# lzzcd001/MeshDiffusion

Hardware: NVIDIA H100
Metric: denoising sample-steps/sec at res-64 (4x64^3), uncond_gen PC sampler (higher is better)
Workload: dtype bf16x3

## Files before the change

### meshdiffusion_b200/csrc/gemm_host.cu

```cuda
#include "gemm_host.h"
#include "elementwise.cuh"
#include <cstring>
#include <cstdlib>
#include <mutex>

namespace mdb {

typedef CUresult (*PFN_encodeTiled)(CUtensorMap*, CUtensorMapDataType, cuuint32_t, void*, const cuuint64_t*,
                                    const cuuint64_t*, const cuuint32_t*, const cuuint32_t*, CUtensorMapInterleave,
                                    CUtensorMapSwizzle, CUtensorMapL2promotion, CUtensorMapFloatOOBfill);

static PFN_encodeTiled get_encode() {
  static PFN_encodeTiled fn = nullptr;
  static std::once_flag once;
  std::call_once(once, [] {
    void* f = nullptr;
    cudaDriverEntryPointQueryResult q;
    cudaError_t e = cudaGetDriverEntryPoint("cuTensorMapEncodeTiled", &f, cudaEnableDefault, &q);
    if (e != cudaSuccess || q != cudaDriverEntryPointSuccess || !f)
      throw std::runtime_error("mdb: cuTensorMapEncodeTiled not available (needs an sm_90+ driver)");
    fn = reinterpret_cast<PFN_encodeTiled>(f);
  });
  return fn;
}
// ... 104 lines not shown
  if (by > 16) by = 16;
  if (by > Y) by = Y;
  int rem = 128 / (bx * by);
  int bz = rem < Z ? rem : Z;
  int bb = rem / bz;
  return {bx, by, bz, bb};
}

int plan_splits(int X, int Y, int Z, int B, int N, int cin_total, int taps, Precision prec) {
  const Geometry g = pick_geometry(X, Y, Z);
  const int tiles_m = ((X + g.bx - 1) / g.bx) * ((Y + g.by - 1) / g.by) * ((Z + g.bz - 1) / g.bz) * ((B + g.bb - 1) / g.bb);
  const int block_n = N <= 32 ? 32 : 128;
  const int tiles = tiles_m * ((N + block_n - 1) / block_n);
  const int kprod = ((cin_total + kb_elems(prec) - 1) / kb_elems(prec)) * taps * (prec == kBF16X3 ? 3 : 1);
  if (tiles > 49 || kprod < 48) return 1;
  int S = kPlanSMs / tiles;
  if (S > 16) S = 16;
  if (S > kprod / 8) S = kprod / 8;
  return S < 2 ? 1 : S;
}

void GemmOp::enable_splits(int S, float* scratch) {
  if (S <= 1) return;
  if (p.ocs != 1 || p.out_fp32 || p.bias_on_m || p.alpha != 1.f || p.res_fp32)
    throw std::runtime_error("mdb: split-K is only wired for plain NDHWC conv outputs");
  if (p.osx != (long long)p.N * parts(prec) || (p.rsx && p.rsx != (long long)p.N * parts(prec)))
    throw std::runtime_error("mdb: split-K needs dense [B][V][N] output / residual");
  splits = S;
  p.splits = S;
  p.partial = scratch;
  p.split_stride = (long long)p.Bn * p.X * p.Y * p.Z * p.N;
}

GemmOp::~GemmOp() {
  if (d_loads) cudaFree(d_loads);
  if (d_ks0) cudaFree(d_ks0);
  if (d_wpacked && owns_w) cudaFree(d_wpacked);
}

static long long physical_strides(bool split, long long lo_off, long long& sx, long long& sy, long long& sz, long long& sb) {
  if (!split) return 0;
  sx *= 2; sy *= 2; sz *= 2; sb *= 2;
  return lo_off;
}

void GemmOp::set_output_strided(Precision pr, int X, int Y, int Z, int B, int N, void* out, long long osx,
                                long long osy, long long osz, long long osb, bool out_fp32, long long lo_off) {
  prec = pr;
  geo = pick_geometry(X, Y, Z);
  if (geo.bx * geo.by * geo.bz * geo.bb != kBlockM) throw std::runtime_error("mdb: unsupported tile geometry");
  if (geo.bb > 1 && (geo.bx * geo.by * geo.bz) % 32 != 0)
    throw std::runtime_error("mdb: multi-sample tiles need a multiple of 32 rows per sample");
  if (geo.bb > 4) throw std::runtime_error("mdb: at most 4 samples per tile");
  p.bx = geo.bx; p.by = geo.by; p.bz = geo.bz; p.bb = geo.bb;
  p.X = X; p.Y = Y; p.Z = Z; p.Bn = B;
  p.tx = (X + geo.bx - 1) / geo.bx; p.ty = (Y + geo.by - 1) / geo.by;
  p.tz = (Z + geo.bz - 1) / geo.bz; p.tb = (B + geo.bb - 1) / geo.bb;
  p.N = N;
  block_n = N <= 32 ? 32 : 128;
  p.n_tiles_n = (N + block_n - 1) / block_n;
  p.out = out;
  p.osx = osx; p.osy = osy; p.osz = osz; p.osb = osb;
  p.out_fp32 = out_fp32 ? 1 : 0;
  p.out_lo_off = physical_strides(prec == kBF16X3 && !out_fp32, lo_off >= 0 ? lo_off : osx, p.osx, p.osy, p.osz, p.osb);
  p.alpha = 1.f;
  p.ocs = 1;
  p.kb_elems = kb_elems(prec);
// ... 267 lines not shown
    p.b_explicit_k = 1;
    p.b_lo_k = (int)b_lo_off;
  }
  if (!b_from_act) p.b_batched = 0;
  p.n_loads = (int)loads.size();
  if (p.splits < 1) p.splits = 1;
  {
    a_slot_need = 0;
    nk_max = 0;
    p.n_segs = 0;
    p.total_groups = 0;
    size_t i = 0;
    while (i < loads.size()) {
      size_t j = i;
      while (j < loads.size() && loads[j].nk == loads[i].nk && loads[j].rows == loads[i].rows && loads[j].jrows == loads[i].jrows) ++j;
      if (p.n_segs >= kMaxSegs) throw std::runtime_error("mdb: too many pipeline segments");
      GemmSeg sg{};
      sg.n_groups = (int)(j - i); sg.nk = loads[i].nk;
      sg.a_bytes = loads[i].rows * kRowBytes;
      sg.a_stride = (sg.a_bytes + 1023) / 1024 * 1024;
      sg.jbytes = loads[i].jrows * kRowBytes;
      const int need = parts(prec) * sg.a_stride;
      if (sg.a_stride > kAStageBytes) throw std::runtime_error("mdb: A box exceeds the slot size");
      if (need > a_slot_need) a_slot_need = need;
      if (sg.nk > nk_max) nk_max = sg.nk;
      p.segs[p.n_segs++] = sg;
      p.total_groups += sg.n_groups;
      i = j;
    }
  }
  if (p.splits > p.total_groups) { p.splits = p.total_groups; splits = p.splits; }
}

void GemmOp::upload(cudaStream_t stream) {
  for (size_t i = 0; i < amaps_.size(); ++i) encode_map(&p.amap[i], prec, amaps_[i]);
  MDB_CUDA_CHECK(cudaMalloc(&d_loads, loads.size() * sizeof(LoadEntry)));
  MDB_CUDA_CHECK(cudaMemcpyAsync(d_loads, loads.data(), loads.size() * sizeof(LoadEntry), cudaMemcpyHostToDevice, stream));
  p.loads = d_loads;
  if (!b_from_act) {
    const long long ktot = 1LL * ksteps * kb_elems(prec) * parts(prec);
    const long long bytes = ktot * p.N * esize(prec);
    MDB_CUDA_CHECK(cudaMalloc(&d_wpacked, bytes));
    owns_w = true;
    bmap_ = b_desc(d_wpacked, ktot, p.N, 1, ktot * esize(prec), bytes);
  }
  encode_map(&p.bmap, prec, bmap_);
  MDB_CUDA_CHECK(cudaStreamSynchronize(stream));
}

void GemmOp::launch(cudaStream_t stream, int B, void* out_override) const {
  GemmParams p = this->p;
  const int smem = pick_slots(p);
  if (B > 0) {
    if (B > this->p.Bn) throw std::runtime_error("mdb: batch exceeds the batch the op was built for");
    p.Bn = B;
    p.tb = (B + p.bb - 1) / p.bb;
  }
  if (out_override) p.out = out_override;
  const int tiles_m = p.tx * p.ty * p.tz * p.tb;
  const int total = tiles_m * p.n_tiles_n * (p.splits > 1 ? p.splits : 1);
  const int grid = total < sm_count() ? total : sm_count();
  if (gnb) {
    if (p.splits > 1) throw std::runtime_error("mdb: GroupNorm-backward epilogue: no split-K");
    p.gnb_drop_thresh = rt_drop_thresh; p.gnb_drop_scale = rt_drop_scale; p.gnb_seed = rt_seed;
  }
  gemm_variant(block_n, prec, gnb).launch(p, grid, smem, stream);
  if (p.splits > 1) {
    SplitReduceArgs a{};
    a.partial = p.partial; a.split_stride = p.split_stride; a.splits = p.splits;
    a.bias = p.bias; a.rowbias = p.rowbias; a.rowbias_ld = p.rowbias_ld;
    a.res = p.res; a.res_batch_stride = p.rsb;
    a.out = p.out; a.stats = p.stats; a.voxels = (long long)p.X * p.Y * p.Z; a.N = p.N; a.prec = prec;
    if (prec == kBF16X3) a.res_batch_stride = p.rsb / 2;
    launch_split_reduce(a, p.Bn, stream);
  }
}

}
```

### meshdiffusion_b200/csrc/gemm_host.h

```cpp
#pragma once
#include <cuda.h>
#include <cuda_runtime.h>
#include <stdint.h>
#include <string>
#include <vector>
#include <stdexcept>
#include "act_format.cuh"
#include "gemm_tc.cuh"

namespace mdb {

#define MDB_CUDA_CHECK(expr)                                                                         \
  do {                                                                                               \
    cudaError_t _e = (expr);                                                                         \
    if (_e != cudaSuccess)                                                                           \
      throw std::runtime_error(std::string("CUDA error ") + cudaGetErrorString(_e) + " at " + __FILE__ + ":" + \
                               std::to_string(__LINE__) + " (" #expr ")");                           \
  } while (0)

inline int kb_elems(Precision p) { return kRowBytes / esize(p); }

struct Act {
  void* ptr = nullptr;
  int C = 0, X = 0, Y = 0, Z = 0, B = 0;
// ... 7 lines not shown
  const float* ptr = nullptr;
  long long sn = 0, sc = 0, st = 0;
  int cvalid = 0;
  int ndiv = 0;
  long long sn_hi = 0;
  int cdiv = 0;
  long long sc_hi = 0;
};

struct Geometry { int bx, by, bz, bb; };
Geometry pick_geometry(int X, int Y, int Z);

struct MapDesc {
  void* base = nullptr;
  int rank = 0;
  uint64_t dims[5] = {}, strides[4] = {};
  uint32_t box[5] = {};
};
MapDesc act_map(const Act& a, Precision prec, int part, Geometry box, int sub = 1, int px = 0, int py = 0, int pz = 0);

class GemmOp {
 public:
  GemmParams p{};
  Precision prec = kBF16;
  int block_n = 128;
  int splits = 1;
  std::vector<LoadEntry> loads;
  std::vector<WSrc> wsrcs;
  int ksteps = 0;
  LoadEntry* d_loads = nullptr;
  int* d_ks0 = nullptr;
  void* d_wpacked = nullptr;
  bool owns_w = false;
  double flops = 0;
  std::string name;

  ~GemmOp();
  GemmOp() = default;
  GemmOp(const GemmOp&) = delete;
  GemmOp& operator=(const GemmOp&) = delete;

  void set_output(Precision prec, int X, int Y, int Z, int B, int N, void* out, long long ldc, bool out_fp32);
  void set_output_strided(Precision prec, int X, int Y, int Z, int B, int N, void* out, long long osx, long long osy,
                          long long osz, long long osb, bool out_fp32, long long lo_off = -1);
  int add_amap(const Act& a, int halo_rows_y, int sub_stride = 1, int px = 0, int py = 0, int pz = 0, int part = 0);
  void add_load_x(int tm_hi, int tm_lo, int nk, int rows, int jrows, int dx, int dy, int dz, int c0, int wsrc, int wc0,
                  int tap0, int tapj);
  int add_wsrc(const WSrc& w) { wsrcs.push_back(w); return (int)wsrcs.size() - 1; }

  void add_conv(const std::vector<Act>& srcs, const float* w_oidhw, int ksize, int stride);
  void add_conv_w(const std::vector<Act>& srcs, const WSrc& w, int ksize, int stride);
  void add_conv_up2(const Act& src, const float* w8, int px, int py, int pz);
  void add_conv_dgrad(const Act& dy, const float* w_oidhw, int cin_total, int ksize);
  void add_pointwise(const std::vector<Act>& srcs, const float* w, bool w_in_out);
  void add_pointwise_w(const std::vector<Act>& srcs, const WSrc* w);

  void set_b_activation(void* ptr, int K, int N, int batch, long long row_stride_elems, long long batch_stride_elems);

  void set_bias(const float* bias, bool on_m = false) { p.bias = bias; p.bias_on_m = on_m ? 1 : 0; }
  void set_rowbias(const float* rb, long long ld) { p.rowbias = rb; p.rowbias_ld = ld; }
  void set_out_col_stride(long long ocs) { p.ocs = ocs; }
  void set_residual(const void* res, long long ldr, long long batch_stride, bool fp32);
  void set_stats(long long* stats) { p.stats = stats; }
  void set_gn_backward(const void* x0, long long ld0, int c0, const void* x1, long long ld1, const void* consts, int silu, float* part);
  long long gnb_rows() const { return 1LL * p.tx * p.ty * p.tz * p.tb * p.bb; }
  int gnb_tiles_per_batch_tile() const { return p.tx * p.ty * p.tz; }
  int gnb_bb() const { return p.bb; }
  bool gnb = false;
  int rt_drop_thresh = 0; float rt_drop_scale = 1.f; unsigned long long rt_seed = 0;
  void set_alpha(float a) { p.alpha = a; }
  void enable_splits(int S, float* scratch);

  void finalize();
  void upload(cudaStream_t stream);
  void repack(cudaStream_t stream);
  void launch(cudaStream_t stream, int B = -1, void* out_override = nullptr) const;
  double fill_bytes(int B = -1) const;
  void slots(int& a_slots, int& b_slots, int& smem_bytes) const;

 private:
  Geometry geo{};
  bool b_from_act = false;
  int a_slot_need = 0;
  int nk_max = 0;
  int pick_slots(GemmParams& q) const;
  long long b_lo_off = 0;
  std::vector<MapDesc> amaps_;
  MapDesc bmap_;
  MapDesc b_desc(void* ptr, long long K, int N, int batch, long long row_stride_bytes, long long batch_stride_bytes) const;
};

int sm_count();
constexpr int kPlanSMs = 132;
void encode_map(CUtensorMap* m, Precision prec, const MapDesc& d);
int plan_splits(int X, int Y, int Z, int B, int N, int cin_total, int taps, Precision prec);

}
```

### meshdiffusion_b200/csrc/gemm_tc.cuh

```cuda
#pragma once
#include "ptx.cuh"
#include "act_format.cuh"
#include "gn_stats.cuh"

namespace mdb {

constexpr int kBlockM = 128;
constexpr int kRowBytes = 128;
constexpr int kAStageRows = 160;
constexpr int kAStageBytes = kAStageRows * kRowBytes;
constexpr int kMaxLoads = 2048;
constexpr int kMaxAMaps = 16;
constexpr int kGemmThreads = 384;
constexpr int kEpiThreads = 256;

struct __align__(16) LoadEntry {
  uint8_t tmap;
  uint8_t nk;
  uint8_t rows;
  uint8_t jrows;
  int8_t dx, dy, dz;
  uint8_t wsrc;
  uint16_t c0;
  uint16_t wc0;
  uint8_t tap0;
  uint8_t tapj;
  uint8_t tmap_lo;
  uint8_t pad;
};
static_assert(sizeof(LoadEntry) == 16, "LoadEntry must be 16 bytes");

struct GemmSeg {
  int n_groups;
  int nk;
  int a_bytes;
  int a_stride;
  int jbytes;
};
constexpr int kMaxSegs = 8;

struct GemmParams {
  CUtensorMap amap[kMaxAMaps];
  CUtensorMap bmap;
  const LoadEntry* loads;
  int n_loads;
  int n_segs;
  GemmSeg segs[kMaxSegs];
  int bx, by, bz, bb;
  int X, Y, Z, Bn;
  int tx, ty, tz, tb;
  int n_tiles_n;
  int N;
  int b_batched;
  int splits;
  int total_groups;
  float* partial;
  long long split_stride;
  int batch_fastest;
  int kb_elems;
  int b_explicit_k;
  int b_kstep;
  int b_lo_k;
  int n_aslots, a_slot_bytes, n_bslots, b_slot_bytes;
  long long out_lo_off, res_lo_off;
  void* out;
  long long osx, osy, osz, osb;
  long long ocs;
  int out_fp32;
  const float* bias;
  int bias_on_m;
  const float* rowbias;
  long long rowbias_ld;
  const void* res;
  long long rsx, rsy, rsz, rsb;
  int res_fp32;
  float alpha;
  long long* stats;
  const void* res1;
  long long r1sx, r1sy, r1sz, r1sb;
  long long res1_lo_off;
  int res_c0;
  const float4* gnb_c;
  int gnb_silu;
  int gnb_drop_thresh; float gnb_drop_scale; unsigned long long gnb_seed;
  float* gnb_part;
};

constexpr int kMaxSlots = 8;
constexpr int kMaxDynSmem = 232448;
template <int BLOCK_N, bool kWholeTile = false>
struct GemmCfg {
  static constexpr int kBTileBytes = BLOCK_N * kRowBytes;
  static constexpr int kStatsFloats = 24 * BLOCK_N;
  static constexpr int kStageCols = (kWholeTile || BLOCK_N < 64) ? BLOCK_N : 64;
  static constexpr int kStageRounds = BLOCK_N / kStageCols;
  static_assert(kStageRounds <= 2, "the epilogue stages at most two rounds");
  static constexpr int kAccPitch = kStageCols + 4;
  static constexpr int kAccFloats = kBlockM * kAccPitch;
  static constexpr int kFixedBytes = 1024 + kAccFloats * 4 + kStatsFloats * 4 + 4 * kMaxSlots * 8;
};
constexpr int kRegsProducer = 40, kRegsConsumer = 232;

__device__ __forceinline__ uint64_t kdesc(uint32_t saddr) { return make_wgmma_desc(saddr, 16, 1024); }

template <int OFF>
__device__ __forceinline__ void colsum_butterfly(float (&s)[32], float (&ss)[32], int lane) {
  const bool hi = (lane & OFF) != 0;
#pragma unroll
  for (int i = 0; i < OFF; ++i) {
    const float send_s = hi ? s[i] : s[i + OFF];
    const float send_q = hi ? ss[i] : ss[i + OFF];
    const float keep_s = hi ? s[i + OFF] : s[i];
    const float keep_q = hi ? ss[i + OFF] : ss[i];
    s[i] = keep_s + __shfl_xor_sync(0xffffffffu, send_s, OFF);
    ss[i] = keep_q + __shfl_xor_sync(0xffffffffu, send_q, OFF);
  }
  if constexpr (OFF > 1) colsum_butterfly<OFF / 2>(s, ss, lane);
}

template <Precision P>
__device__ __forceinline__ void add_res_chunk(const uint4 (&buf)[8], float (&v)[32]) {
  constexpr int E = kVecElems<P>, NV = 32 / E;
#pragma unroll
  for (int i = 0; i < NV; ++i) {
    float r[E];
    decode_vec<P>(buf[i], buf[P == kBF16X3 ? NV + i : i], r);
#pragma unroll
    for (int j = 0; j < E; ++j) v[E * i + j] += r[j];
  }
}

template <int BLOCK_N, Precision P, bool GNB>
__global__ void __launch_bounds__(kGemmThreads, 1) gemm_tc_kernel(const __grid_constant__ GemmParams p) {
  static_assert(!(GNB && P == kTF32), "the GroupNorm-backward epilogue is built for bf16 / split-bf16 operands");
  using Cfg = GemmCfg<BLOCK_N, GNB>;
// ... 65 lines not shown
          const GemmSeg& seg = p.segs[sg];
          for (int g = 0; g < seg.n_groups; ++g, ++gi) {
            if (gi < g_lo || gi >= g_hi) {
              kcol += seg.nk * p.b_kstep;
              ++l;
              continue;
            }
            const uint4 raw = __ldg(reinterpret_cast<const uint4*>(p.loads + l));
            const LoadEntry& en = reinterpret_cast<const LoadEntry&>(raw);
            mbar_wait(a_empty + 8 * as, aph ^ 1);
            if (elect_one()) {
              const uint32_t abase = a_ring + as * a_slot, bar = a_full + 8 * as;
              mbar_expect_tx(bar, kParts * seg.a_bytes);
              tma_load_5d(&p.amap[en.tmap], bar, abase, en.c0, x0 + en.dx, y0 + en.dy, z0 + en.dz, b0);
              if constexpr (P == kBF16X3) tma_load_5d(&p.amap[en.tmap_lo], bar, abase + seg.a_stride, en.c0, x0 + en.dx, y0 + en.dy, z0 + en.dz, b0);
            }
            __syncwarp();
            if (++as == (uint32_t)NA) { as = 0; aph ^= 1; }
            int kc = (P == kBF16X3 && p.b_explicit_k) ? (int)en.wc0 : kcol;
            for (int j = 0; j < seg.nk; ++j) {
              mbar_wait(b_empty + 8 * bs, bph ^ 1);
              if (elect_one()) {
                const uint32_t bbase = b_ring + bs * b_slot, bar = b_full + 8 * bs;
                mbar_expect_tx(bar, kParts * Cfg::kBTileBytes);
                tma_load_3d(&p.bmap, bar, bbase, kc, n0, bcoord);
                if constexpr (P == kBF16X3) tma_load_3d(&p.bmap, bar, bbase + Cfg::kBTileBytes, kc + p.b_lo_k, n0, bcoord);
              }
              __syncwarp();
              kc += p.b_kstep;
              if (++bs == (uint32_t)NB) { bs = 0; bph ^= 1; }
            }
            kcol += seg.nk * p.b_kstep;
            ++l;
          }
        }
      }
    }
  } else {
    setmaxnreg_inc<kRegsConsumer>();
    const int wg = (warp - 4) >> 2;
    const int wt = threadIdx.x & 127;
    const int q = warp & 3;
    const int half = (warp - 4) >> 2;
    constexpr int kChunks = BLOCK_N / 32;
    constexpr int kChunkStep = kChunks >= 2 ? 2 : 1;
    const int row = q * 32 + lane;
    const int et = threadIdx.x - 128;
    const int rows_per_b = p.bx * p.by * p.bz;
    const int seg = row / rows_per_b;
    int it = 0;
    int staged_n0 = -1, staged_b0 = -1, bias_buf = 0;
    int want_cols = 0;
    if constexpr (GNB) {
      want_cols = (p.stats != nullptr || p.gnb_part != nullptr) ? 1 : 0;
      asm volatile("" : "+r"(want_cols));
    }
    uint32_t as = 0, aph = 0, bs = 0, bph = 0;
    for (int tile = first_tile; tile < total_tiles; tile += tile_step, ++it) {
      const int vit = it;
      constexpr int kAccRegs = kParts * BLOCK_N / 2;
      float acc[kAccRegs];
      float (&acc_hi)[BLOCK_N / 2] = *reinterpret_cast<float (*)[BLOCK_N / 2]>(acc);
#pragma unroll
      for (int i = 0; i < kAccRegs; ++i) acc[i] = 0.f;
      {
        int gi = 0, g_lo, g_hi;
        split_range(tile, g_lo, g_hi);
        int prev_b = -1, prev_a = -1;
        const uint32_t a_row0 = (uint32_t)wg * 64 * kRowBytes;
        for (int sg = 0; sg < p.n_segs; ++sg) {
          const GemmSeg& sgm = p.segs[sg];
          for (int g = 0; g < sgm.n_groups; ++g, ++gi) {
            if (gi < g_lo || gi >= g_hi) continue;
            mbar_wait(a_full + 8 * as, aph);
            const uint32_t abase = a_ring + as * a_slot + a_row0;
            for (int j = 0; j < sgm.nk; ++j) {
              mbar_wait(b_full + 8 * bs, bph);
              const uint64_t ad = kdesc(abase + j * sgm.jbytes);
              const uint64_t bd = kdesc(b_ring + bs * b_slot);
              wgmma_fence();
              if constexpr (P == kBF16X3) {
                const uint64_t adl = kdesc(abase + sgm.a_stride + j * sgm.jbytes);
#pragma unroll
                for (int k = 0; k < kRowBytes / 32; ++k) wgmma_kmajor<2 * BLOCK_N, false>(acc, ad + 2 * k, bd + 2 * k, 1u);
                wgmma_fence();
#pragma unroll
                for (int k = 0; k < kRowBytes / 32; ++k) wgmma_kmajor<BLOCK_N, false>(acc_hi, adl + 2 * k, bd + 2 * k, 1u);
              } else {
#pragma unroll
                for (int k = 0; k < kRowBytes / 32; ++k) wgmma_kmajor<BLOCK_N, P == kTF32>(acc, ad + 2 * k, bd + 2 * k, 1u);
              }
              wgmma_commit();
              wgmma_wait<1>();
              if (wt == 0) {
                if (prev_b >= 0) mbar_arrive(b_empty + 8 * prev_b);
                if (prev_a >= 0) mbar_arrive(a_empty + 8 * prev_a);
              }
              prev_b = (int)bs;
              prev_a = j + 1 == sgm.nk ? (int)as : -1;
              if (++bs == (uint32_t)NB) { bs = 0; bph ^= 1; }
            }
            if (++as == (uint32_t)NA) { as = 0; aph ^= 1; }
          }
        }
        wgmma_wait<0>();
        fence_operands(acc);
        if (wt == 0) {
          if (prev_b >= 0) mbar_arrive(b_empty + 8 * prev_b);
          if (prev_a >= 0) mbar_arrive(a_empty + 8 * prev_a);
        }
        if constexpr (P == kBF16X3) {
#pragma unroll
          for (int i = 0; i < BLOCK_N / 2; ++i) acc[i] += acc[BLOCK_N / 2 + i];
        }
      }
      int x0, y0, z0, b0, n0;
      decode(tile, x0, y0, z0, b0, n0);
      int r = row;
      const int xl = r % p.bx; r /= p.bx;
      const int yl = r % p.by; r /= p.by;
      const int zl = r % p.bz; r /= p.bz;
      const int xg = x0 + xl, yg = y0 + yl, zg = z0 + zl, bg = b0 + r;
      const bool valid = (xg < p.X) && (yg < p.Y) && (zg < p.Z) && (bg < p.Bn);
      const long long ooff = xg * p.osx + yg * p.osy + zg * p.osz + bg * p.osb;
      const long long roff = xg * p.rsx + yg * p.rsy + zg * p.rsz + bg * p.rsb;

      constexpr int kRoundRegs = Cfg::kStageCols / 2;
      auto stage = [&]() {
        const int w4 = (warp & 3), srow = wg * 64 + w4 * 16 + (lane >> 2), scol = 2 * (lane & 3);
#pragma unroll
        for (int j = 0; j < Cfg::kStageCols / 8; ++j) {
          *reinterpret_cast<float2*>(s_acc + srow * Cfg::kAccPitch + 8 * j + scol) = make_float2(acc[4 * j], acc[4 * j + 1]);
          *reinterpret_cast<float2*>(s_acc + (srow + 8) * Cfg::kAccPitch + 8 * j + scol) = make_float2(acc[4 * j + 2], acc[4 * j + 3]);
        }
      };
      named_bar_sync(2, kEpiThreads);
      stage();
      if constexpr (Cfg::kStageRounds > 1) {
#pragma unroll
// ... 21 lines not shown
      uint4 rbuf[8];
      auto prefetch_res = [&](int ch) {
        const int nbp = n0 + ch * 32;
        if (!(p.res && valid && p.ocs == 1 && nbp + 32 <= p.N)) return;
        if constexpr (GNB) {
          const bool second = p.res1 && nbp >= p.res_c0;
          const __nv_bfloat16* base = reinterpret_cast<const __nv_bfloat16*>(second ? p.res1 : p.res);
          const long long off = second ? xg * p.r1sx + yg * p.r1sy + zg * p.r1sz + bg * p.r1sb + (nbp - p.res_c0) : roff + nbp;
          const uint4* rp = reinterpret_cast<const uint4*>(base + off);
#pragma unroll
          for (int i = 0; i < 4; ++i) rbuf[i] = __ldg(rp + i);
          if constexpr (P == kBF16X3) {
            const uint4* rl = reinterpret_cast<const uint4*>(base + off + (second ? p.res1_lo_off : p.res_lo_off));
#pragma unroll
            for (int i = 0; i < 4; ++i) rbuf[4 + i] = __ldg(rl + i);
          }
          return;
        }
        if (P == kTF32 || p.res_fp32) {
          const uint4* rp = reinterpret_cast<const uint4*>(reinterpret_cast<const float*>(p.res) + roff + nbp);
#pragma unroll
          for (int i = 0; i < 8; ++i) rbuf[i] = __ldg(rp + i);
        } else {
          const uint4* rp = reinterpret_cast<const uint4*>(reinterpret_cast<const __nv_bfloat16*>(p.res) + roff + nbp);
#pragma unroll
          for (int i = 0; i < 4; ++i) rbuf[i] = __ldg(rp + i);
          if constexpr (P == kBF16X3) {
            const uint4* rl = reinterpret_cast<const uint4*>(reinterpret_cast<const __nv_bfloat16*>(p.res) + roff + nbp + p.res_lo_off);
#pragma unroll
            for (int i = 0; i < 4; ++i) rbuf[4 + i] = __ldg(rl + i);
          }
        }
      };
      const int ch0 = kChunkStep == 2 ? half : 0;
      const bool active = kChunkStep == 2 || half == 0;
      if (active) prefetch_res(ch0);

      constexpr int kRoundChunks = Cfg::kStageCols / 32;
#pragma unroll 1
      for (int rnd = 0; rnd < Cfg::kStageRounds; ++rnd) {
        if (rnd > 0) {
          named_bar_sync(2, kEpiThreads);
          stage();
        }
        named_bar_sync(2, kEpiThreads);

#pragma unroll 1
        for (int ch = ch0 + rnd * kRoundChunks; ch < (rnd + 1) * kRoundChunks && active; ch += kChunkStep) {
          uint32_t rr[32];
          {
            const float4* src = reinterpret_cast<const float4*>(s_acc + row * Cfg::kAccPitch + (ch - rnd * kRoundChunks) * 32);
#pragma unroll
            for (int i = 0; i < 8; ++i) {
              const float4 t = src[i];
              rr[4 * i] = __float_as_uint(t.x); rr[4 * i + 1] = __float_as_uint(t.y);
              rr[4 * i + 2] = __float_as_uint(t.z); rr[4 * i + 3] = __float_as_uint(t.w);
            }
          }
          const int nb = n0 + ch * 32;
          if (nb >= p.N) continue;
          if (splits > 1) {
            if (valid) {
              float* pp = p.partial + (long long)(tile % splits) * p.split_stride + (P == kBF16X3 ? (ooff >> 1) : ooff) + nb;
              if (nb + 32 <= p.N) {
#pragma unroll
                for (int i = 0; i < 8; ++i)
                  reinterpret_cast<float4*>(pp)[i] = make_float4(__uint_as_float(rr[4 * i]), __uint_as_float(rr[4 * i + 1]),
                                                                 __uint_as_float(rr[4 * i + 2]), __uint_as_float(rr[4 * i + 3]));
              } else {
                for (int i = 0; i < 32; ++i) if (nb + i < p.N) pp[i] = __uint_as_float(rr[i]);
              }
            }
            continue;
          }
          const bool full = (nb + 32 <= p.N) && (p.ocs == 1);
          float v[32];
          const float mbias = (p.bias && p.bias_on_m && valid) ? __ldg(p.bias + xg) : 0.f;
          const float* sb = s_bias + (seg < 4 ? seg : 0) * BLOCK_N + ch * 32;
// ... 2 lines not shown
          float q2[GNB ? 32 : 1];
          if constexpr (GNB) {
            if (valid) {
              const float4* cc = p.gnb_c + static_cast<long long>(bg) * p.N + nb;
              unsigned long long hsh[8];
              if (p.gnb_drop_thresh > 0) {
                const unsigned long long e4 = (unsigned long long)((((static_cast<long long>(bg) * p.Z + zg) * p.Y + yg) * p.X + xg) * p.N + nb) >> 2;
#pragma unroll
                for (int i = 0; i < 8; ++i) hsh[i] = drop_hash64(p.gnb_seed, e4 + i);
              }
#pragma unroll
              for (int i = 0; i < 32; ++i) {
                const float4 kc = __ldg(cc + i);
                const __nv_bfloat16 xb = reinterpret_cast<const __nv_bfloat16*>(rbuf)[i];
                float xv = __bfloat162float(xb);
                if constexpr (P == kBF16X3) xv += __bfloat162float(reinterpret_cast<const __nv_bfloat16*>(rbuf + 4)[i]);
                float d = v[i];
                if (p.gnb_drop_thresh > 0) {
                  const unsigned r16 = (unsigned)((hsh[i >> 2] >> (16 * (i & 3))) & 0xFFFFu);
                  d = r16 >= (unsigned)p.gnb_drop_thresh ? d * p.gnb_drop_scale : 0.f;
                }
                if (p.gnb_silu) {
                  const float h = fmaf(xv, kc.x, kc.y);
                  d *= P == kBF16X3 ? dsilu_ex2_half(h) : dsilu_tanh_half(h);
                }
                v[i] = d;
                q2[i] = d * fmaf(xv, kc.z, kc.w);
              }
            } else {
#pragma unroll
              for (int i = 0; i < 32; ++i) q2[i] = 0.f;
            }
          }
          if (!GNB && p.res && valid) {
            if (P == kTF32 || p.res_fp32) {
              if (full) {
                add_res_chunk<kTF32>(rbuf, v);
              } else {
                const float* rp = reinterpret_cast<const float*>(p.res) + roff + nb;
                for (int i = 0; i < 32; ++i) if (nb + i < p.N) v[i] += rp[i];
              }
            } else {
              if (full) {
                add_res_chunk<P>(rbuf, v);
              } else {
                const ActElem<P>* rp = reinterpret_cast<const ActElem<P>*>(p.res) + roff + nb;
                for (int i = 0; i < 32; ++i) if (nb + i < p.N) v[i] += load_split<P>(rp + i, p.res_lo_off);
              }
            }
          }
          if (ch + kChunkStep < kChunks) prefetch_res(ch + kChunkStep);
          if (valid) {
            if (p.out_fp32) {
              float* op = reinterpret_cast<float*>(p.out) + ooff + nb;
              if (full) {
#pragma unroll
                for (int i = 0; i < 8; ++i) reinterpret_cast<float4*>(op)[i] = make_float4(v[4 * i], v[4 * i + 1], v[4 * i + 2], v[4 * i + 3]);
              } else {
                for (int i = 0; i < 32; ++i) if (nb + i < p.N) op[i * p.ocs] = v[i];
              }
            } else {
              ActElem<P>* op = reinterpret_cast<ActElem<P>*>(p.out) + ooff + nb;
              if (full) {
                constexpr int E = kVecElems<P>;
#pragma unroll
                for (int i = 0; i < 32 / E; ++i) store_vec<P>(op + E * i, p.out_lo_off * (long long)sizeof(ActElem<P>), v + E * i);
              } else {
                for (int i = 0; i < 32; ++i) if (nb + i < p.N) store_split<P>(op + i * p.ocs, p.out_lo_off, v[i]);
              }
            }
          }
          if (GNB ? (want_cols != 0) : (p.stats != nullptr)) {
            float s[32], ss[32];
#pragma unroll
            for (int i = 0; i < 32; ++i) {
              const float t = valid ? v[i] : 0.f;
              s[i] = t; ss[i] = GNB ? q2[GNB ? i : 0] : t * t;
            }
            colsum_butterfly<16>(s, ss, lane);
            s_part[(q * 2 + 0) * BLOCK_N + ch * 32 + lane] = s[0];
            s_part[(q * 2 + 1) * BLOCK_N + ch * 32 + lane] = ss[0];
          }
        }
      }
      if constexpr (GNB) {
        if (p.gnb_part && splits == 1) {
          named_bar_sync(1, kEpiThreads);
          const int warps_per_seg = rows_per_b >= 128 ? 4 : rows_per_b / 32;
          for (int i = et; i < p.bb * BLOCK_N; i += kEpiThreads) {
            const int sg = i / BLOCK_N, c = i % BLOCK_N;
            const int n = n0 + c;
            if (mt_of_tile < tiles_m && n < p.N) {
              float ts = 0.f, tq = 0.f;
              for (int w = sg * warps_per_seg; w < (sg + 1) * warps_per_seg; ++w) {
                ts += s_part[(w * 2 + 0) * BLOCK_N + c];
                tq += s_part[(w * 2 + 1) * BLOCK_N + c];
              }
              float* dst = p.gnb_part + ((static_cast<long long>(mt_of_tile) * p.bb + sg) * p.N + n) * 2;
              dst[0] = ts; dst[1] = tq;
            }
          }
        }
      }
      if (!GNB && p.stats && splits == 1) {
        named_bar_sync(1, kEpiThreads);
        const int warps_per_seg = rows_per_b >= 128 ? 4 : rows_per_b / 32;
        for (int i0 = 0; i0 < p.bb * BLOCK_N; i0 += kEpiThreads) {
          const int i = i0 + et;
          const int sg = i / BLOCK_N, c = i % BLOCK_N;
          const int bgl = b0 + sg, n = n0 + c;
          if (i < p.bb * BLOCK_N && bgl < p.Bn && n < p.N) {
            float ts = 0.f, tq = 0.f;
            for (int w = sg * warps_per_seg; w < (sg + 1) * warps_per_seg; ++w) {
              ts += s_part[(w * 2 + 0) * BLOCK_N + c];
              tq += s_part[(w * 2 + 1) * BLOCK_N + c];
            }
            long long* dst = p.stats + (static_cast<long long>(bgl) * p.N + n) * kStatWords;
            stat_add(dst, ts);
            stat_add(dst + 2, tq);
          }
        }
      }
    }
  }
}

}
```

### meshdiffusion_b200/csrc/ptx.cuh

```cuda
#pragma once
#include <cuda.h>
#include <cuda_runtime.h>
#include <cuda_bf16.h>
#include <stdint.h>
#include <stdio.h>

namespace mdb {

__device__ __forceinline__ uint32_t smem_u32(const void* p) {
  return static_cast<uint32_t>(__cvta_generic_to_shared(p));
}

__device__ __forceinline__ void mbar_init(uint32_t bar, uint32_t count) {
  asm volatile("mbarrier.init.shared::cta.b64 [%0], %1;" ::"r"(bar), "r"(count) : "memory");
}
__device__ __forceinline__ void fence_barrier_init() {
  asm volatile("fence.mbarrier_init.release.cluster;" ::: "memory");
}
__device__ __forceinline__ void fence_proxy_async() {
  asm volatile("fence.proxy.async.shared::cta;" ::: "memory");
}
__device__ __forceinline__ void mbar_expect_tx(uint32_t bar, uint32_t bytes) {
  asm volatile("mbarrier.arrive.expect_tx.shared::cta.b64 _, [%0], %1;" ::"r"(bar), "r"(bytes) : "memory");
}
// ... 3 lines not shown
__device__ __forceinline__ void mbar_wait(uint32_t bar, uint32_t parity) {
  asm volatile(
      "{\n\t.reg .pred p;\n\t.reg .u32 n;\n\tmov.u32 n, 0;\n"
      "MDB_WAIT:\n\t"
      "mbarrier.try_wait.parity.shared::cta.b64 p, [%0], %1;\n\t"
      "@p bra MDB_DONE;\n\t"
      "add.u32 n, n, 1;\n\t"
      "setp.lt.u32 p, n, 16777216;\n\t"
      "@p bra MDB_WAIT;\n\t"
      "trap;\n"
      "MDB_DONE:\n\t}"
      :: "r"(bar), "r"(parity) : "memory");
}

__device__ __forceinline__ void tma_prefetch_desc(const void* desc) {
  asm volatile("prefetch.tensormap [%0];" ::"l"(reinterpret_cast<uint64_t>(desc)) : "memory");
}
__device__ __forceinline__ void tma_load_5d(const void* desc, uint32_t bar, uint32_t dst, int c0, int c1, int c2,
                                            int c3, int c4) {
  asm volatile(
      "cp.async.bulk.tensor.5d.shared::cluster.global.mbarrier::complete_tx::bytes"
      " [%0], [%1, {%3, %4, %5, %6, %7}], [%2];"
      :
      : "r"(dst), "l"(reinterpret_cast<uint64_t>(desc)), "r"(bar), "r"(c0), "r"(c1), "r"(c2), "r"(c3), "r"(c4)
      : "memory");
}
__device__ __forceinline__ void tma_load_3d(const void* desc, uint32_t bar, uint32_t dst, int c0, int c1, int c2) {
  asm volatile(
      "cp.async.bulk.tensor.3d.shared::cluster.global.mbarrier::complete_tx::bytes"
      " [%0], [%1, {%3, %4, %5}], [%2];"
      :
      : "r"(dst), "l"(reinterpret_cast<uint64_t>(desc)), "r"(bar), "r"(c0), "r"(c1), "r"(c2)
      : "memory");
}

__device__ __forceinline__ uint64_t make_wgmma_desc(uint32_t saddr, uint32_t lbo_bytes, uint32_t sbo_bytes) {
  return static_cast<uint64_t>((saddr & 0x3FFFFu) >> 4) | (static_cast<uint64_t>((lbo_bytes >> 4) & 0x3FFFu) << 16) |
         (static_cast<uint64_t>((sbo_bytes >> 4) & 0x3FFFu) << 32) | (static_cast<uint64_t>(1) << 62);
}
__device__ __forceinline__ void wgmma_fence() { asm volatile("wgmma.fence.sync.aligned;" ::: "memory"); }
__device__ __forceinline__ void wgmma_commit() { asm volatile("wgmma.commit_group.sync.aligned;" ::: "memory"); }
template <int N>
__device__ __forceinline__ void wgmma_wait() { asm volatile("wgmma.wait_group.sync.aligned %0;" ::"n"(N) : "memory"); }
template <int N>
__device__ __forceinline__ void fence_operands(float (&d)[N]) {
#pragma unroll
  for (int i = 0; i < N; ++i) asm volatile("" : "+f"(d[i])::"memory");
}

template <int TA, int TB>
__device__ __forceinline__ void wgmma_m64n32k16_bf16(float (&d)[16], uint64_t a, uint64_t b, uint32_t scale_d) {
  asm volatile(
      "{\n\t.reg .pred p;\n\tsetp.ne.b32 p, %18, 0;\n\t"
      "wgmma.mma_async.sync.aligned.m64n32k16.f32.bf16.bf16 "
      "{%0, %1, %2, %3, %4, %5, %6, %7, %8, %9, %10, %11, %12, %13, %14, %15}, "
      "%16, %17, p, 1, 1, %19, %20;\n\t}"
      : "+f"(d[0]), "+f"(d[1]), "+f"(d[2]), "+f"(d[3]), "+f"(d[4]), "+f"(d[5]), "+f"(d[6]), "+f"(d[7]), "+f"(d[8]), "+f"(d[9]), "+f"(d[10]), "+f"(d[11]), "+f"(d[12]), "+f"(d[13]), "+f"(d[14]), "+f"(d[15])
      : "l"(a), "l"(b), "r"(scale_d), "n"(TA), "n"(TB));
}
__device__ __forceinline__ void wgmma_m64n32k8_tf32(float (&d)[16], uint64_t a, uint64_t b, uint32_t scale_d) {
  asm volatile(
      "{\n\t.reg .pred p;\n\tsetp.ne.b32 p, %18, 0;\n\t"
      "wgmma.mma_async.sync.aligned.m64n32k8.f32.tf32.tf32 "
      "{%0, %1, %2, %3, %4, %5, %6, %7, %8, %9, %10, %11, %12, %13, %14, %15}, "
      "%16, %17, p, 1, 1;\n\t}"
      : "+f"(d[0]), "+f"(d[1]), "+f"(d[2]), "+f"(d[3]), "+f"(d[4]), "+f"(d[5]), "+f"(d[6]), "+f"(d[7]), "+f"(d[8]), "+f"(d[9]), "+f"(d[10]), "+f"(d[11]), "+f"(d[12]), "+f"(d[13]), "+f"(d[14]), "+f"(d[15])
// ... 80 lines not shown
```

Measured before the change: 36.68.

## Move conv GEMM epilogue residual loads and output stores to TMA via B-ring slots

For bf16/bf16x3 GEMMs with BLOCK_N 128 and no split-K, the producer warp TMA-loads residual tiles into free B-ring slots. The consumers read them from swizzled shared memory, write the encoded bf16 hi/lo output back into the same slot, and issue 5D TMA bulk stores. Slot release is deferred until the bulk reads complete. This replaces per-thread global residual prefetches and scattered stores with bulk async transfers, at the cost of extra B-ring pressure, more synchronisation, and re-encoding tensor maps whenever the output pointer or batch size changes. It also adds an optional globaltimer tracing path that is compiled out by default.

Result: faster. 38.06, median of 6 (+3.8%).

```diff
diff --git a/meshdiffusion_b200/csrc/gemm_host.cu b/meshdiffusion_b200/csrc/gemm_host.cu
--- a/meshdiffusion_b200/csrc/gemm_host.cu
+++ b/meshdiffusion_b200/csrc/gemm_host.cu
@@ -160,7 +160,31 @@
   p.split_stride = (long long)p.Bn * p.X * p.Y * p.Z * p.N;
 }
 
+#ifdef MDB_EPI_TRACE
+std::vector<const GemmOp*>& trace_registry() {
+  static std::vector<const GemmOp*> ops;
+  return ops;
+}
+extern "C" int mdb_epi_trace_read(int i, char* name, int name_cap, unsigned long long* out) {
+  auto& ops = trace_registry();
+  if (i < 0 || i >= (int)ops.size()) return -1;
+  snprintf(name, name_cap, "%s", ops[i]->name.c_str());
+  if (cudaMemcpy(out, ops[i]->d_trace, sizeof(unsigned long long) * kTraceCtas * kTraceTiles * kTraceStamps,
+                 cudaMemcpyDeviceToHost) != cudaSuccess) return -2;
+  return kTraceCtas * kTraceTiles * kTraceStamps;
+}
+extern "C" int mdb_epi_trace_dims(int* ctas, int* tiles, int* stamps) {
+  *ctas = kTraceCtas; *tiles = kTraceTiles; *stamps = kTraceStamps;
+  return 0;
+}
+#endif
+
 GemmOp::~GemmOp() {
+#ifdef MDB_EPI_TRACE
+  auto& ops = trace_registry();
+  for (size_t i = 0; i < ops.size(); ++i) if (ops[i] == this) { ops.erase(ops.begin() + i); break; }
+  if (d_trace) cudaFree(d_trace);
+#endif
   if (d_loads) cudaFree(d_loads);
   if (d_ks0) cudaFree(d_ks0);
   if (d_wpacked && owns_w) cudaFree(d_wpacked);
@@ -494,8 +518,55 @@
   if (p.splits > p.total_groups) { p.splits = p.total_groups; splits = p.splits; }
 }
 
+bool GemmOp::epi_tma_ok(const GemmParams& p) const {
+  if (gnb || block_n != 128 || prec == kTF32 || p.splits > 1 || p.ocs != 1 || p.out_fp32) return false;
+  if (p.res && (p.res_fp32 || p.batch_fastest)) return false;
+  const long long es = esize(prec);
+  auto aligned = [&](const void* base, long long lo_off, long long sx, long long sy, long long sz, long long sb) {
+    const uintptr_t a = reinterpret_cast<uintptr_t>(base);
+    return a % 16 == 0 && (lo_off * es) % 16 == 0 && (sx * es) % 16 == 0 && (sy * es) % 16 == 0 && (sz * es) % 16 == 0 &&
+           (sb * es) % 16 == 0;
+  };
+  if (!aligned(p.out, prec == kBF16X3 ? p.out_lo_off : 0, p.osx, p.osy, p.osz, p.osb)) return false;
+  if (p.res && !aligned(p.res, prec == kBF16X3 ? p.res_lo_off : 0, p.rsx, p.rsy, p.rsz, p.rsb)) return false;
+  return true;
+}
+
+static MapDesc epi_map(const void* base, Precision prec, int part, long long lo_off, const GemmParams& q, int B, long long sx,
+                       long long sy, long long sz, long long sb) {
+  const long long es = esize(prec);
+  MapDesc m;
+  m.rank = 5;
+  m.base = const_cast<char*>(static_cast<const char*>(base)) + (long long)part * lo_off * es;
+  m.dims[0] = q.N; m.dims[1] = q.X; m.dims[2] = q.Y; m.dims[3] = q.Z; m.dims[4] = B;
+  const long long st[4] = {sx * es, sy * es, sz * es, sb * es};
+  long long prev = es * q.N;
+  for (int i = 0; i < 4; ++i) {
+    m.strides[i] = (uint64_t)(m.dims[i + 1] == 1 ? prev : st[i]);
+    prev = (long long)m.strides[i] * (long long)m.dims[i + 1];
+  }
+  m.box[0] = kRowBytes / es; m.box[1] = q.bx; m.box[2] = q.by; m.box[3] = q.bz; m.box[4] = q.bb;
+  return m;
+}
+
+void GemmOp::encode_epi_maps(GemmParams& q, int B) const {
+  for (int part = 0; part < parts(prec); ++part) {
+    encode_map(&q.omap[part], prec, epi_map(q.out, prec, part, q.out_lo_off, q, B, q.osx, q.osy, q.osz, q.osb));
+    if (q.res) encode_map(&q.rmap[part], prec, epi_map(q.res, prec, part, q.res_lo_off, q, B, q.rsx, q.rsy, q.rsz, q.rsb));
+  }
+}
+
 void GemmOp::upload(cudaStream_t stream) {
   for (size_t i = 0; i < amaps_.size(); ++i) encode_map(&p.amap[i], prec, amaps_[i]);
+  p.epi_tma = epi_tma_ok(p) ? 1 : 0;
+  if (p.epi_tma && p.out) encode_epi_maps(p, p.Bn);
+#ifdef MDB_EPI_TRACE
+  if (getenv("MDB_EPI_TRACE_PER_THREAD")) p.epi_tma = 0;
+  MDB_CUDA_CHECK(cudaMalloc(&d_trace, sizeof(unsigned long long) * kTraceCtas * kTraceTiles * kTraceStamps));
+  MDB_CUDA_CHECK(cudaMemset(d_trace, 0, sizeof(unsigned long long) * kTraceCtas * kTraceTiles * kTraceStamps));
+  p.trace = d_trace;
+  trace_registry().push_back(this);
+#endif
   MDB_CUDA_CHECK(cudaMalloc(&d_loads, loads.size() * sizeof(LoadEntry)));
   MDB_CUDA_CHECK(cudaMemcpyAsync(d_loads, loads.data(), loads.size() * sizeof(LoadEntry), cudaMemcpyHostToDevice, stream));
   p.loads = d_loads;
@@ -519,6 +590,10 @@
     p.tb = (B + p.bb - 1) / p.bb;
   }
   if (out_override) p.out = out_override;
+  if (p.epi_tma && (out_override || p.Bn != this->p.Bn)) {
+    p.epi_tma = epi_tma_ok(p) ? 1 : 0;
+    if (p.epi_tma) encode_epi_maps(p, p.Bn);
+  }
   const int tiles_m = p.tx * p.ty * p.tz * p.tb;
   const int total = tiles_m * p.n_tiles_n * (p.splits > 1 ? p.splits : 1);
   const int grid = total < sm_count() ? total : sm_count();
diff --git a/meshdiffusion_b200/csrc/gemm_host.h b/meshdiffusion_b200/csrc/gemm_host.h
--- a/meshdiffusion_b200/csrc/gemm_host.h
+++ b/meshdiffusion_b200/csrc/gemm_host.h
@@ -63,6 +63,9 @@
   int* d_ks0 = nullptr;
   void* d_wpacked = nullptr;
   bool owns_w = false;
+#ifdef MDB_EPI_TRACE
+  unsigned long long* d_trace = nullptr;
+#endif
   double flops = 0;
   std::string name;
 
@@ -115,6 +118,8 @@
   int a_slot_need = 0;
   int nk_max = 0;
   int pick_slots(GemmParams& q) const;
+  bool epi_tma_ok(const GemmParams& q) const;
+  void encode_epi_maps(GemmParams& q, int B) const;
   long long b_lo_off = 0;
   std::vector<MapDesc> amaps_;
   MapDesc bmap_;
@@ -122,6 +127,9 @@
 };
 
 int sm_count();
+#ifdef MDB_EPI_TRACE
+std::vector<const GemmOp*>& trace_registry();
+#endif
 constexpr int kPlanSMs = 132;
 void encode_map(CUtensorMap* m, Precision prec, const MapDesc& d);
 int plan_splits(int X, int Y, int Z, int B, int N, int cin_total, int taps, Precision prec);
diff --git a/meshdiffusion_b200/csrc/gemm_tc.cuh b/meshdiffusion_b200/csrc/gemm_tc.cuh
--- a/meshdiffusion_b200/csrc/gemm_tc.cuh
+++ b/meshdiffusion_b200/csrc/gemm_tc.cuh
@@ -42,6 +42,12 @@
 struct GemmParams {
   CUtensorMap amap[kMaxAMaps];
   CUtensorMap bmap;
+  CUtensorMap omap[2];
+  CUtensorMap rmap[2];
+  int epi_tma;
+#ifdef MDB_EPI_TRACE
+  unsigned long long* trace;
+#endif
   const LoadEntry* loads;
   int n_loads;
   int n_segs;
@@ -101,6 +107,18 @@
 };
 constexpr int kRegsProducer = 40, kRegsConsumer = 232;
 
+template <int BLOCK_N, Precision P, bool GNB>
+constexpr bool kHasTmaEpi = !GNB && BLOCK_N == 128 && P != kTF32;
+constexpr int kEpiBoxBytes = 64 * 2 * kBlockM;
+static_assert(kEpiBoxBytes == GemmCfg<128>::kBTileBytes, "an epilogue box is one weight tile");
+
+#ifdef MDB_EPI_TRACE
+constexpr int kTraceCtas = 16, kTraceTiles = 64, kTraceStamps = 6;
+#define MDB_STAMP(k) do { if (trace_row && et == 0) trace_row[k] = globaltimer(); } while (0)
+#else
+#define MDB_STAMP(k) do { } while (0)
+#endif
+
 __device__ __forceinline__ uint64_t kdesc(uint32_t saddr) { return make_wgmma_desc(saddr, 16, 1024); }
 
 template <int OFF>
@@ -232,6 +250,26 @@
             }
             kcol += seg.nk * p.b_kstep;
             ++l;
+          }
+        }
+        if constexpr (kHasTmaEpi<BLOCK_N, P, GNB>) {
+          if (p.epi_tma) {
+            for (int rnd = 0; rnd < Cfg::kStageRounds; ++rnd) {
+              mbar_wait(b_empty + 8 * bs, bph ^ 1);
+              if (elect_one()) {
+                const uint32_t bbase = b_ring + bs * b_slot, bar = b_full + 8 * bs;
+                const int c = n0 + rnd * Cfg::kStageCols;
+                if (p.res && c < p.N) {
+                  mbar_expect_tx(bar, kParts * kEpiBoxBytes);
+                  tma_load_5d(&p.rmap[0], bar, bbase, c, x0, y0, z0, b0);
+                  if constexpr (P == kBF16X3) tma_load_5d(&p.rmap[1], bar, bbase + kEpiBoxBytes, c, x0, y0, z0, b0);
+                } else {
+                  mbar_arrive(bar);
+                }
+              }
+              __syncwarp();
+              if (++bs == (uint32_t)NB) { bs = 0; bph ^= 1; }
+            }
           }
         }
       }
@@ -256,8 +294,22 @@
       asm volatile("" : "+r"(want_cols));
     }
     uint32_t as = 0, aph = 0, bs = 0, bph = 0;
+    int epi_pend = -1;
     for (int tile = first_tile; tile < total_tiles; tile += tile_step, ++it) {
       const int vit = it;
+#ifdef MDB_EPI_TRACE
+      unsigned long long* trace_row = (p.trace && (int)blockIdx.x < kTraceCtas && it < kTraceTiles)
+                                          ? p.trace + ((long long)blockIdx.x * kTraceTiles + it) * kTraceStamps : nullptr;
+      bool first_k = true;
+#endif
+      if constexpr (kHasTmaEpi<BLOCK_N, P, GNB>) {
+        if (et == 0 && epi_pend >= 0) {
+          bulk_wait_read<0>();
+          mbar_arrive(b_empty + 8 * epi_pend);
+          mbar_arrive(b_empty + 8 * epi_pend);
+          epi_pend = -1;
+        }
+      }
       constexpr int kAccRegs = kParts * BLOCK_N / 2;
       float acc[kAccRegs];
       float (&acc_hi)[BLOCK_N / 2] = *reinterpret_cast<float (*)[BLOCK_N / 2]>(acc);
@@ -276,6 +328,9 @@
             const uint32_t abase = a_ring + as * a_slot + a_row0;
             for (int j = 0; j < sgm.nk; ++j) {
               mbar_wait(b_full + 8 * bs, bph);
+#ifdef MDB_EPI_TRACE
+              if (first_k) { MDB_STAMP(5); first_k = false; }
+#endif
               const uint64_t ad = kdesc(abase + j * sgm.jbytes);
               const uint64_t bd = kdesc(b_ring + bs * b_slot);
               wgmma_fence();
@@ -305,6 +360,7 @@
         }
         wgmma_wait<0>();
         fence_operands(acc);
+        MDB_STAMP(0);
         if (wt == 0) {
           if (prev_b >= 0) mbar_arrive(b_empty + 8 * prev_b);
           if (prev_a >= 0) mbar_arrive(a_empty + 8 * prev_a);
@@ -392,9 +448,10 @@
           }
         }
       };
+      const bool tma_epi = kHasTmaEpi<BLOCK_N, P, GNB> && p.epi_tma != 0;
       const int ch0 = kChunkStep == 2 ? half : 0;
       const bool active = kChunkStep == 2 || half == 0;
-      if (active) prefetch_res(ch0);
+      if (active && !tma_epi) prefetch_res(ch0);
 
       constexpr int kRoundChunks = Cfg::kStageCols / 32;
 #pragma unroll 1
@@ -404,6 +461,17 @@
           stage();
         }
         named_bar_sync(2, kEpiThreads);
+        if (rnd == 0) MDB_STAMP(1);
+        int eslot_i = 0;
+        uint8_t* eslot = nullptr;
+        if constexpr (kHasTmaEpi<BLOCK_N, P, GNB>) {
+          if (tma_epi) {
+            eslot_i = (int)bs;
+            eslot = smem + NA * p.a_slot_bytes + bs * p.b_slot_bytes;
+            mbar_wait(b_full + 8 * bs, bph);
+            if (++bs == (uint32_t)NB) { bs = 0; bph ^= 1; }
+          }
+        }
 
 #pragma unroll 1
         for (int ch = ch0 + rnd * kRoundChunks; ch < (rnd + 1) * kRoundChunks && active; ch += kChunkStep) {
@@ -472,7 +540,17 @@
               for (int i = 0; i < 32; ++i) q2[i] = 0.f;
             }
           }
-          if (!GNB && p.res && valid) {
+          const int chr = ch - rnd * kRoundChunks;
+          auto eoff = [&](int i) { return row * 128 + (((4 * chr + i) ^ (row & 7)) << 4); };
+          if (!GNB && p.res && valid && tma_epi) {
+            uint4 buf[8];
+#pragma unroll
+            for (int i = 0; i < 4; ++i) {
+              buf[i] = *reinterpret_cast<const uint4*>(eslot + eoff(i));
+              buf[4 + i] = P == kBF16X3 ? *reinterpret_cast<const uint4*>(eslot + kEpiBoxBytes + eoff(i)) : buf[i];
+            }
+            add_res_chunk<P>(buf, v);
+          } else if (!GNB && p.res && valid) {
             if (P == kTF32 || p.res_fp32) {
               if (full) {
                 add_res_chunk<kTF32>(rbuf, v);
@@ -489,8 +567,15 @@
               }
             }
           }
-          if (ch + kChunkStep < kChunks) prefetch_res(ch + kChunkStep);
-          if (valid) {
+          if (!tma_epi && ch + kChunkStep < kChunks) prefetch_res(ch + kChunkStep);
+          if (tma_epi) {
+#pragma unroll
+            for (int i = 0; i < 4; ++i) {
+              const uint4 h = bf16x8_encode(v + 8 * i);
+              *reinterpret_cast<uint4*>(eslot + eoff(i)) = h;
+              if constexpr (P == kBF16X3) *reinterpret_cast<uint4*>(eslot + kEpiBoxBytes + eoff(i)) = bf16x8_encode_lo(h, v + 8 * i);
+            }
+          } else if (valid) {
             if (p.out_fp32) {
               float* op = reinterpret_cast<float*>(p.out) + ooff + nb;
               if (full) {
@@ -522,6 +607,28 @@
             s_part[(q * 2 + 1) * BLOCK_N + ch * 32 + lane] = ss[0];
           }
         }
+        if constexpr (kHasTmaEpi<BLOCK_N, P, GNB>) {
+          if (tma_epi) {
+            fence_proxy_async();
+            named_bar_sync(2, kEpiThreads);
+            if (et == 0) {
+              const int c = n0 + rnd * Cfg::kStageCols;
+              const uint32_t src = b_ring + eslot_i * b_slot;
+              if (c < p.N) {
+                tma_store_5d(&p.omap[0], src, c, x0, y0, z0, b0);
+                if constexpr (P == kBF16X3) tma_store_5d(&p.omap[1], src + kEpiBoxBytes, c, x0, y0, z0, b0);
+              }
+              bulk_commit();
+              if (epi_pend >= 0) {
+                bulk_wait_read<1>();
+                mbar_arrive(b_empty + 8 * epi_pend);
+                mbar_arrive(b_empty + 8 * epi_pend);
+              }
+              epi_pend = eslot_i;
+            }
+          }
+        }
+        MDB_STAMP(2 + rnd);
       }
       if constexpr (GNB) {
         if (p.gnb_part && splits == 1) {
@@ -561,6 +668,10 @@
           }
         }
       }
+      MDB_STAMP(4);
+    }
+    if constexpr (kHasTmaEpi<BLOCK_N, P, GNB>) {
+      if (et == 0 && epi_pend >= 0) bulk_wait<0>();
     }
   }
 }
diff --git a/meshdiffusion_b200/csrc/ptx.cuh b/meshdiffusion_b200/csrc/ptx.cuh
--- a/meshdiffusion_b200/csrc/ptx.cuh
+++ b/meshdiffusion_b200/csrc/ptx.cuh
@@ -59,6 +59,23 @@
       :
       : "r"(dst), "l"(reinterpret_cast<uint64_t>(desc)), "r"(bar), "r"(c0), "r"(c1), "r"(c2)
       : "memory");
+}
+__device__ __forceinline__ void tma_store_5d(const void* desc, uint32_t src, int c0, int c1, int c2, int c3, int c4) {
+  asm volatile(
+      "cp.async.bulk.tensor.5d.global.shared::cta.bulk_group [%0, {%2, %3, %4, %5, %6}], [%1];"
+      :
+      : "l"(reinterpret_cast<uint64_t>(desc)), "r"(src), "r"(c0), "r"(c1), "r"(c2), "r"(c3), "r"(c4)
+      : "memory");
+}
+__device__ __forceinline__ void bulk_commit() { asm volatile("cp.async.bulk.commit_group;" ::: "memory"); }
+template <int N>
+__device__ __forceinline__ void bulk_wait_read() { asm volatile("cp.async.bulk.wait_group.read %0;" ::"n"(N) : "memory"); }
+template <int N>
+__device__ __forceinline__ void bulk_wait() { asm volatile("cp.async.bulk.wait_group %0;" ::"n"(N) : "memory"); }
+__device__ __forceinline__ unsigned long long globaltimer() {
+  unsigned long long t;
+  asm volatile("mov.u64 %0, %%globaltimer;" : "=l"(t));
+  return t;
 }
 
 __device__ __forceinline__ uint64_t make_wgmma_desc(uint32_t saddr, uint32_t lbo_bytes, uint32_t sbo_bytes) {
```
